# AsherBond/0-kno-vectorx

Hardware: AMD Instinct MI355X
Metric: header_range_256 proofs/sec (higher is better)
Workload: dtype u64 (Goldilocks) / u8 (hashes)

## Files before the change

### 0-kno-vectorx_amd/csrc/air.cuh

```cuda
#pragma once
#include <hip/hip_runtime.h>
#include <stdint.h>

#include <type_traits>
#include <vector>

#include "air_bus.cuh"
#include "gl.cuh"
#include "glh.h"

struct vx_ctx;
typedef int32_t (*gen_aux_fn)(vx_ctx*, const uint64_t* trace, int log_n, const uint64_t* chal, const uint64_t* pub, uint64_t* aux, uint64_t* aux_pub);

template <int R>
struct FpN {
    static constexpr int LANES = R;
    uint64_t v[R];
    __device__ __forceinline__ FpN operator+(const FpN& o) const {
        FpN r;
#pragma unroll
        for (int j = 0; j < R; ++j) r.v[j] = gl_add(v[j], o.v[j]);
        return r;
    }
    __device__ __forceinline__ FpN operator-(const FpN& o) const {
        FpN r;
#pragma unroll
        for (int j = 0; j < R; ++j) r.v[j] = gl_sub(v[j], o.v[j]);
        return r;
    }
    __device__ __forceinline__ FpN operator*(const FpN& o) const {
        FpN r;
#pragma unroll
        for (int j = 0; j < R; ++j) r.v[j] = gl_mul(v[j], o.v[j]);
        return r;
    }
// ... 47 lines not shown
        acc[0] = acc[0] * alpha[0] + c;
        acc[1] = acc[1] * alpha[1] + c;
    }
    VX_HD void transition(F c) { constraint(c * z_last); }
    VX_HD void first_row(F c) { constraint(c * l_first); }
    VX_HD void last_row(F c) { constraint(c * l_last); }
    VX_HD void constraint_x2(const X2<F>& e) {
        constraint(e.a);
        constraint(e.b);
    }
    VX_HD Gate open(F g) { return Gate{g}; }
    VX_HD void gated(Gate& G, F e) { constraint(G.g * e); }
    VX_HD void close(Gate&) {}
};

template <int R>
struct Consumer<FpN<R>> {
    using F = FpN<R>;
    struct Gate {
        gl_acc a0[R], a1[R];
        F g;
    };
    gl_acc acc0[R], acc1[R];
    const uint64_t* apow;
    int k;
    F z_last, l_first, l_last;
    __device__ __forceinline__ void init(const uint64_t* apow_) {
        apow = apow_, k = 0;
#pragma unroll
        for (int j = 0; j < R; ++j) gl_acc_zero(acc0[j]), gl_acc_zero(acc1[j]);
    }
    __device__ __forceinline__ void push(gl_acc* a0, gl_acc* a1, const F& c) {
        const int ku = __builtin_amdgcn_readfirstlane(k);
        const uint64_t p0 = apow[2 * ku], p1 = apow[2 * ku + 1];
#pragma unroll
        for (int j = 0; j < R; ++j) {
            gl_mac(a0[j], c.v[j], p0);
            gl_mac(a1[j], c.v[j], p1);
        }
        k = ku + 1;
    }
    __device__ __forceinline__ void constraint(const F& c) { push(acc0, acc1, c); }
    __device__ __forceinline__ void transition(const F& c) { constraint(c * z_last); }
    __device__ __forceinline__ void first_row(const F& c) { constraint(c * l_first); }
    __device__ __forceinline__ void last_row(const F& c) { constraint(c * l_last); }
    __device__ __forceinline__ void constraint_x2(const X2<F>& e) {
        constraint(e.a);
        constraint(e.b);
    }
    __device__ __forceinline__ Gate open(const F& g) {
        Gate G;
// ... 25 lines not shown
    int k = 0;
    void constraint(CountF) { ++k; }
    void transition(CountF) { ++k; }
    void first_row(CountF) { ++k; }
    void last_row(CountF) { ++k; }
    void constraint_x2(const X2<CountF>&) { k += 2; }
    Gate open(CountF) { return {}; }
    void gated(Gate&, CountF) { ++k; }
    void close(Gate&) {}
};
struct CountRow {
    CountF operator[](int) const { return {}; }
};

template <int R>
struct RowViewN {
    const uint64_t* base;
    size_t stride, i[R];
    __device__ __forceinline__ FpN<R> operator[](int col) const {
        const uint64_t* c = base + (size_t)col * stride;
        FpN<R> r;
#pragma unroll
        for (int j = 0; j < R; ++j) r.v[j] = c[i[j]];
        return r;
    }
};

template <class F, class Row, class Cn>
struct BusConstraints {
    static constexpr int UNROLL = 1;
    const Row& loc;
    Cn& c;
    int at;
    X2<F> hsum;
    VX_HD X2<F> helper() {
        const X2<F> h{loc[at], loc[at + 1]};
        at += 2, hsum = hsum + h;
        return h;
    }
    VX_HD void put(const F& ma, const X2<F>& da, const F& mb, const X2<F>& db) { c.constraint_x2(helper() * da * db - db * ma - da * mb); }
    VX_HD void pair(const F& m, const X2<F>& da, const X2<F>& db) { c.constraint_x2(helper() * da * db - (da + db) * m); }
    VX_HD void single(const F& m, const X2<F>& d) { c.constraint_x2(helper() * d - m); }
};
template <class Air, class F, class Row, class Cn>
VX_HD void bus_constraints(const Row& loc, const Row& nxt, const F* per, const F* pub, const F* chal, const F* apub, Cn& c) {
    static_assert(Air::AUX == 2 * Air::N_HELP + 2 && Air::AUXPUB == 1 && Air::CHAL == 4, "air.cuh: helpers, then one running sum");
// ... 62 lines not shown
```

### 0-kno-vectorx_amd/csrc/vx_core.hip

```cpp
#include <stdarg.h>
#include <stdlib.h>
#include <stdio.h>
#include <string.h>

#include "gl.cuh"
#include <dlfcn.h>

#include "vx_internal.h"

__attribute__((constructor)) static void vx_runtime_env() { setenv("GPU_MAX_HW_QUEUES", "16", 0); }

extern "C" int32_t vx_table_streams_mode(const char* table_streams, const char* hw_queues) {
    if (table_streams && strcmp(table_streams, "own") == 0) return VX_TABLE_STREAMS_OWN;
    if (table_streams && strcmp(table_streams, "shared") == 0) return VX_TABLE_STREAMS_SHARED;
    if (!hw_queues) return VX_TABLE_STREAMS_SHARED;
    char* end = nullptr;
    const long q = strtol(hw_queues, &end, 10);
    if (end == hw_queues || *end || q < 1) return VX_TABLE_STREAMS_OWN;
    return q <= 4 ? VX_TABLE_STREAMS_SHARED : VX_TABLE_STREAMS_OWN;
}

hipError_t vx_wait(vx_ctx* ctx) {
    if (ctx->table_streams != VX_TABLE_STREAMS_SHARED) return hipStreamSynchronize(ctx->stream);
    const hipError_t e = hipEventRecord(ctx->ev_wait, ctx->stream);
// ... 118 lines not shown
        ctx->scratch_n = n;
    }
    *out = ctx->scratch;
    return VX_OK;
}

extern "C" {

const char* vx_backend_name(void) { return "hip-gfx950"; }

static int32_t ctx_create(int device, vx_ctx* parent, vx_ctx** out) {
    if (!out) return VX_ERR_ARG;
    *out = nullptr;
    int n_dev = 0;
    if (hipGetDeviceCount(&n_dev) != hipSuccess || n_dev == 0 || device < 0 || device >= n_dev) return VX_ERR_DEVICE;
    vx_ctx* ctx = new vx_ctx();
    ctx->device = device;
    ctx->scratch = nullptr;
    ctx->scratch_n = 0;
    ctx->pinned = nullptr;
    ctx->pinned_n = 0;
    ctx->table_streams = parent ? parent->table_streams : vx_table_streams_mode(getenv("VX_TABLE_STREAMS"), getenv("GPU_MAX_HW_QUEUES"));
    ctx->stream_owned = !(parent && ctx->table_streams == VX_TABLE_STREAMS_SHARED);
    const char* sm = getenv("VX_SYNC_MODE");
    const char m = sm ? sm[0] : 'b';
    (void)hipSetDevice(device);
    (void)hipSetDeviceFlags(m == 's' ? hipDeviceScheduleSpin : m == 'y' ? hipDeviceScheduleYield : hipDeviceScheduleBlockingSync);
    (void)hipGetLastError();
    hipError_t se = hipSetDevice(device);
    if (se == hipSuccess && !ctx->stream_owned) ctx->stream = parent->stream;
    else if (se == hipSuccess) {
        const char* sp = getenv("VX_STREAM_PRIO");
        int least = 0, greatest = 0;
        if (sp && sp[0] == '1' && hipDeviceGetStreamPriorityRange(&least, &greatest) == hipSuccess && least != greatest)
            se = hipStreamCreateWithPriority(&ctx->stream, hipStreamDefault, parent ? least : greatest);
        else se = hipStreamCreate(&ctx->stream);
    }
    if (se != hipSuccess || hipEventCreate(&ctx->ev0) != hipSuccess || hipEventCreate(&ctx->ev1) != hipSuccess ||
        hipEventCreateWithFlags(&ctx->ev_wait, hipEventDisableTiming | (m == 's' || m == 'y' ? 0 : hipEventBlockingSync)) != hipSuccess) {
        delete ctx;
        return VX_ERR_DEVICE;
    }
    int32_t rc = make_powtab(ctx, glh::ROOT_2_32, &ctx->tw_fwd);
    if (rc == VX_OK) rc = make_powtab(ctx, glh::inv(glh::ROOT_2_32), &ctx->tw_inv);
    if (rc == VX_OK) {
        std::vector<uint64_t> f(2048), b(2048);
// ... 212 lines not shown
```

### 0-kno-vectorx_amd/csrc/vx_internal.h

```cpp
#pragma once
#include <hip/hip_runtime.h>
#include <stdint.h>
#include <map>
#include <string>
#include <vector>

#pragma GCC visibility push(default)
#include "../../include/vx.h"
#pragma GCC visibility pop
#include "glh.h"

#ifndef VX_TAIL_PRIO
#define VX_TAIL_PRIO 1
#endif
#if VX_TAIL_PRIO
#define VX_TAIL_KERNEL_ENTRY() __builtin_amdgcn_s_setprio(3)
#else
#define VX_TAIL_KERNEL_ENTRY() ((void)0)
#endif

struct vx_buf {
    uint64_t* d;
    size_t n;
};

struct PowTab {
    uint64_t* d;
};

enum { VX_TABLE_STREAMS_OWN = 0, VX_TABLE_STREAMS_SHARED = 1 };

struct vx_ctx {
    int device;
    hipStream_t stream;
    bool stream_owned;
    int table_streams;
    hipEvent_t ev0, ev1;
    hipEvent_t ev_wait;
    std::string err;
    PowTab tw_fwd, tw_inv;
    uint64_t *w12_fwd, *w12_inv;
    std::map<uint64_t, PowTab> shift_tabs;
    std::map<int, uint64_t*> tw2;
    uint64_t* scratch;
    size_t scratch_n;
    void* pinned;
    size_t pinned_n;
    std::map<size_t, std::vector<void*>> pool_free;
    std::map<void*, size_t> pool_live;
    vx_ctx* side = nullptr;
    std::map<uint64_t, uint64_t*> periodic_cache;
};
vx_ctx* vx_side_ctx(vx_ctx* ctx);
hipError_t vx_wait(vx_ctx* ctx);
void* vx_pool_alloc(vx_ctx* ctx, size_t bytes);
void vx_pool_free(vx_ctx* ctx, void* p);
void vx_pool_trim(vx_ctx* ctx);
int32_t vx_fail(vx_ctx* ctx, int32_t code, const char* fmt, ...);

// ... 118 lines not shown
```

### 0-kno-vectorx_amd/csrc/vx_stark.hip

```cpp
#include <string.h>

#include <map>
#include <mutex>

#include <array>

#include "air_list.h"
#include "air_program.h"
#include "bus_aux_prog.cuh"
#include "stark_proof.h"
#include "vx_internal.h"

namespace sp = stark_proof;

__device__ __forceinline__ uint64_t root_pow_f(const uint64_t* tw, uint64_t e, int log_s) {
    uint64_t E = (e << (32 - log_s)) & 0xFFFFFFFFULL;
    uint64_t r = tw[4096 + (E >> 22)];
    if (log_s > 10) r = gl_mul(r, tw[2048 + ((E >> 11) & 2047)]);
    if (log_s > 21) r = gl_mul(r, tw[E & 2047]);
    return r;
}

struct QuotArgs {
    const uint64_t* lde;
    uint64_t* q_out;
    int log_N, rate_bits;
    uint64_t shift, last, n_inv;
    uint64_t alpha[2];
    uint64_t zh_inv[8];
    uint64_t zh[8];
    const uint64_t* periodic;
    const uint64_t* pub;
    const uint64_t* tw;
    const uint64_t* apow;
    uint64_t chal[8];
    uint64_t apub[8];
};

#ifndef VX_Q_WAVES
#define VX_Q_WAVES 4
#endif
#ifndef VX_Q_WAVES_MAX
#define VX_Q_WAVES_MAX 8
#endif
#ifndef VX_Q_BLOCK
#define VX_Q_BLOCK 256
#endif
constexpr int QB = VX_Q_BLOCK;
template <class Air, int R>
__global__ __launch_bounds__(QB) __attribute__((amdgpu_waves_per_eu(VX_Q_WAVES, VX_Q_WAVES_MAX))) void k_quotient(QuotArgs a) {
    using F = FpN<R>;
    const size_t N = (size_t)1 << a.log_N;
    const size_t i0 = blockIdx.x * (size_t)(QB * R) + threadIdx.x;
    const size_t step = (size_t)1 << a.rate_bits;
    Consumer<F> c;
    c.init(a.apow);
    RowViewN<R> loc{a.lde, N, {}}, nxt{a.lde, N, {}};
    F per[Air::PERIODIC > 0 ? Air::PERIODIC : 1], pub[Air::PUB > 0 ? Air::PUB : 1];
    F chal[Air::CHAL > 0 ? Air::CHAL : 1], apub[Air::AUXPUB > 0 ? 2 * Air::AUXPUB : 1];
// ... 10 lines not shown
        zinv[j] = a.zh_inv[k];
        loc.i[j] = i;
        nxt.i[j] = (i + step) & (N - 1);
        size_t poff = 0;
#pragma unroll
        for (int q = 0; q < Air::PERIODIC; ++q) {
            const size_t plen = (size_t)1 << (Air::plog(q) + a.rate_bits);
            per[q].v[j] = a.periodic[poff + (i & (plen - 1))];
            poff += plen;
        }
    }
#pragma unroll
    for (int q = 0; q < Air::PUB; ++q) pub[q] = F::from(a.pub[q]);
#pragma unroll
    for (int q = 0; q < Air::CHAL; ++q) chal[q] = F::from(a.chal[q]);
#pragma unroll
    for (int q = 0; q < 2 * Air::AUXPUB; ++q) apub[q] = F::from(a.apub[q]);
    Air::template eval<F>(loc, nxt, per, pub, chal, apub, c);
#pragma unroll
    for (int j = 0; j < R; ++j) {
        a.q_out[loc.i[j]] = gl_mul(c.result(0, j), zinv[j]);
        a.q_out[N + loc.i[j]] = gl_mul(c.result(1, j), zinv[j]);
    }
}

struct ProgArgs {
    const uint64_t* code;
    const uint64_t* consts;
    const uint64_t* per_tab;
    int n_code;
};
__global__ __launch_bounds__(QB) void k_quotient_prog(QuotArgs a, ProgArgs p) {
    extern __shared__ uint64_t prog_regs[];
    using F = Fp;
    const size_t N = (size_t)1 << a.log_N;
    const size_t i = (blockIdx.x * (size_t)QB + threadIdx.x) & (N - 1);
    const size_t step = (size_t)1 << a.rate_bits, inext = (i + step) & (N - 1);
    Consumer<F> c;
    c.init(a.apow);
    const uint64_t x = gl_mul(a.shift, root_pow_f(a.tw, i, a.log_N));
    const int kz = (int)(i & (step - 1));
    c.z_last.v[0] = gl_sub(x, a.last);
    const uint64_t zh_n = gl_mul(a.zh[kz], a.n_inv);
    c.l_first.v[0] = gl_mul(zh_n, gl_inv(gl_sub(x, 1)));
    c.l_last.v[0] = gl_mul(gl_mul(zh_n, a.last), gl_inv(gl_sub(x, a.last)));
    uint64_t* R = prog_regs + threadIdx.x;
// ... 142 lines not shown
        const gl2 s1{gl_acc_reduce(sa[r]), gl_acc_reduce(sb[r])};
        gl2 s0 = s1;
        for (int j = 0; j < a.n_q; ++j) {
            const int k = a.n_cols + j;
            s0 = gl2_add(s0, gl2_scale({a.alpha_pow[2 * k], a.alpha_pow[2 * k + 1]}, a.quot_lde[(size_t)j * N + i]));
        }
        const uint64_t x = gl_mul(a.shift, root_pow_f(a.tw, i, a.log_N));
        gl2 t0 = gl2_mul(gl2_sub(s0, a.y0), gl2_inv({gl_sub(x, a.zeta.a), gl_neg(a.zeta.b)}));
        gl2 t1 = gl2_mul(gl2_sub(s1, a.y1), gl2_inv({gl_sub(x, a.zeta_next.a), gl_neg(a.zeta_next.b)}));
        gl2 f = gl2_add(gl2_mul(a.alpha_c, t0), t1);
        a.out[2 * i] = f.a;
        a.out[2 * i + 1] = f.b;
    }
}

struct AirDesc {
    int id, cols, pub, periodic, period_log, exact_log;
    void (*periodic_values)(std::vector<uint64_t>&);
    void (*launch)(QuotArgs&, hipStream_t);
    int (*count)();
    int aux, chal, auxpub;
    int (*plog)(int);
    gen_aux_fn gen_aux;
    const AirProgram* prog = nullptr;
};
template <class Air>
static int count_q() {
    static const int k = [] {
        Consumer<CountF> c;
        CountRow r;
        CountF per[Air::PERIODIC > 0 ? Air::PERIODIC : 1], pub[Air::PUB > 0 ? Air::PUB : 1], chal[Air::CHAL > 0 ? Air::CHAL : 1], apub[Air::AUXPUB > 0 ? 2 * Air::AUXPUB : 1];
        Air::template eval<CountF>(r, r, per, pub, chal, apub, c);
        return c.k;
    }();
    return k;
}
template <class Air>
static void launch_q(QuotArgs& a, hipStream_t s) {
    constexpr int R = Air::QUOT_ROWS_PER_LANE;
    const size_t N = (size_t)1 << a.log_N;
    if (R > 1 && N >= QB * (size_t)R) hipLaunchKernelGGL((k_quotient<Air, R>), dim3((unsigned)(N / (QB * R))), dim3(QB), 0, s, a);
    else hipLaunchKernelGGL((k_quotient<Air, 1>), dim3((unsigned)((N + QB - 1) / QB)), dim3(QB), 0, s, a);
}
template <class Air>
static AirDesc desc() {
    return {Air::ID, Air::COLS, Air::PUB, Air::PERIODIC, Air::PERIOD_LOG, Air::EXACT_LOG, Air::periodic_values, launch_q<Air>, count_q<Air>, Air::AUX, Air::CHAL, Air::AUXPUB, Air::plog, Air::gen_aux};
}
template <class... Airs>
static std::array<AirDesc, sizeof...(Airs)> descs(AirList<Airs...>) { return {{desc<Airs>()...}}; }
static const auto AIRS = descs(VxAirs{});
static std::mutex g_prog_desc_mu;
static std::map<int, AirDesc> g_prog_desc;
static const AirDesc* find_air(int id) {
    for (const AirDesc& d : AIRS)
        if (d.id == id) return &d;
    if (id >= VX_AIR_USER_BASE) {
        const AirProgram* pg = vx_air_program_find(id);
        if (!pg) return nullptr;
        std::lock_guard<std::mutex> lk(g_prog_desc_mu);
        auto it = g_prog_desc.find(id);
        if (it == g_prog_desc.end()) {
            AirDesc d{};
            d.id = id, d.cols = (int)pg->cols, d.pub = (int)pg->pub, d.periodic = (int)pg->plog.size(), d.period_log = pg->period_log, d.prog = pg;
            d.aux = (int)pg->aux, d.chal = (int)pg->chal, d.auxpub = (int)pg->auxpub;
            it = g_prog_desc.emplace(id, d).first;
        }
        return &it->second;
    }
    return nullptr;
// ... 56 lines not shown
}

struct DevMem;
static int32_t quotient_eval_dev(vx_ctx* ctx, const AirDesc* air, int L, int r, const uint64_t* trace_lde, const uint64_t alphas[2],
                                 const uint64_t* public_inputs, size_t n_public, const uint64_t* chal, const uint64_t* apub, uint64_t* qv, DevMem& mem);

extern "C" {

int32_t vx_stark_default_config(vx_stark_config* cfg) {
    if (!cfg) return VX_ERR_ARG;
    cfg->rate_bits = 1;
    cfg->cap_height = 4;
    cfg->num_queries = 84;
    cfg->pow_bits = 16;
    cfg->arity_bits = 4;
    cfg->final_poly_bits = 5;
    return VX_OK;
}

int32_t vx_stark_proof_bound(int air_id, const vx_stark_config* cfg, int log_n, size_t* n_words) {
    const AirDesc* air = find_air(air_id);
    if (!air || !cfg || !n_words || log_n < 2 || cfg->rate_bits < 1) return VX_ERR_ARG;
    *n_words = sp::Shape(air_id, air->cols, air->aux, air->pub, air->auxpub, log_n, *cfg).bound_words();
    return VX_OK;
}

int32_t vx_quotient_eval(vx_ctx* ctx, int air_id, int rate_bits, const vx_buf* trace_lde, int log_n, const uint64_t alphas[2],
                         const uint64_t* public_inputs, size_t n_public, vx_buf* out) {
    if (!ctx || !trace_lde || !alphas || !out) return VX_ERR_ARG;
    const AirDesc* air = find_air(air_id);
    VX_CHECK(air, "quotient eval: unknown AIR id %d", air_id);
    VX_CHECK(air->aux == 0, "quotient eval: AIR %d has an auxiliary round (its challenges are not part of this entry point)", air_id);
    VX_CHECK(rate_bits >= 1 && rate_bits <= 3 && log_n >= 2 && log_n >= air->period_log && log_n + rate_bits <= 27, "quotient eval: bad log_n %d / rate_bits %d", log_n, rate_bits);
    VX_CHECK((int)n_public == air->pub && (n_public == 0 || public_inputs), "quotient eval: AIR %d takes %d public inputs", air_id, air->pub);
    const size_t N = (size_t)1 << (log_n + rate_bits);
    VX_CHECK(trace_lde->n >= N * (size_t)air->cols && out->n >= 2 * N, "quotient eval: buffers too small");
    VX_CHECK(alphas[0] < glh::P && alphas[1] < glh::P, "quotient eval: non-canonical challenge");
    DevMem mem{ctx};
    return quotient_eval_dev(ctx, air, log_n, rate_bits, trace_lde->d, alphas, public_inputs, n_public, nullptr, nullptr, out->d, mem);
}

int32_t vx_quotient_eval_aux(vx_ctx* ctx, int air_id, int rate_bits, const vx_buf* trace_lde, int log_n, const uint64_t alphas[2],
                             const uint64_t* public_inputs, size_t n_public, const uint64_t* challenges, size_t n_challenges,
                             const uint64_t* aux_public, size_t n_aux_public, vx_buf* out) {
    if (!ctx || !trace_lde || !alphas || !out) return VX_ERR_ARG;
    const AirDesc* air = find_air(air_id);
// ... 65 lines not shown
        if (pl <= 6) {
            periodic_on_coset(pv.data() + in_off, pl, r, shift_pow, tab.data() + off);
            VX_HIP(hipMemcpyAsync(d + off, tab.data() + off, m * 8, hipMemcpyHostToDevice, ctx->stream));
        } else {
            uint64_t* tmp = (uint64_t*)vx_pool_alloc(ctx, p * 8);
            if (!tmp) {
                (void)hipFree(d);
                return vx_fail(ctx, VX_ERR_OOM, "stark prove: out of device memory (periodic table)");
            }
            VX_HIP(hipMemcpyAsync(tmp, pv.data() + in_off, p * 8, hipMemcpyHostToDevice, ctx->stream));
            int32_t rc = vx_lde_dev(ctx, tmp, pl, 1, r, shift_pow, VX_LDE_SRC_VALUES, d + off, nullptr);
            VX_HIP(vx_wait(ctx));
            vx_pool_free(ctx, tmp);
            if (rc != VX_OK) {
                (void)hipFree(d);
                return rc;
            }
        }
        off += m, in_off += p;
    }
    VX_HIP(vx_wait(ctx));
    ctx->periodic_cache[key] = d;
    *out = d;
    return VX_OK;
}

static int32_t quotient_eval_dev(vx_ctx* ctx, const AirDesc* air, int L, int r, const uint64_t* trace_lde, const uint64_t alphas[2],
                                 const uint64_t* public_inputs, size_t n_public, const uint64_t* chal, const uint64_t* apub, uint64_t* qv, DevMem& mem) {
    const int LN = L + r;
    const size_t n = (size_t)1 << L;
    const uint64_t g = 7;
    uint64_t* d_pub = mem.alloc(n_public ? n_public : 1);
    VX_CHECK(d_pub, "stark prove: out of device memory (quotient)");
    if (n_public) VX_HIP(hipMemcpyAsync(d_pub, public_inputs, n_public * 8, hipMemcpyHostToDevice, ctx->stream));
    const uint64_t* d_per = nullptr;
    if (air->periodic) VX_TRY(periodic_table_dev(ctx, air, L, r, &d_per));
    {
        QuotArgs qa{};
        qa.lde = trace_lde;
        qa.q_out = qv;
        qa.log_N = LN;
        qa.rate_bits = r;
        qa.shift = g;
        qa.last = glh::inv(glh::root(L));
        qa.n_inv = glh::inv(n % glh::P);
        qa.alpha[0] = alphas[0];
// ... 27 lines not shown
            uint64_t* d_code = nullptr;
            auto it = ctx->periodic_cache.find(key);
            if (it != ctx->periodic_cache.end()) d_code = it->second;
            else {
                std::vector<uint64_t> blob(pg.code);
                blob.insert(blob.end(), pg.consts.begin(), pg.consts.end());
                VX_HIP(hipMalloc((void**)&d_code, blob.size() * 8));
                VX_HIP(hipMemcpyAsync(d_code, blob.data(), blob.size() * 8, hipMemcpyHostToDevice, ctx->stream));
                VX_HIP(vx_wait(ctx));
                ctx->periodic_cache[key] = d_code;
            }
            size_t off = 0;
            for (size_t q = 0; q < pg.plog.size(); ++q) {
                const size_t plen = (size_t)1 << (pg.plog[q] + r);
                per_tab.push_back(off), per_tab.push_back(plen - 1);
                off += plen;
            }
            uint64_t* d_per_tab = mem.alloc(per_tab.size() ? per_tab.size() : 1);
            VX_CHECK(d_per_tab, "stark prove: out of device memory (program tables)");
            if (!per_tab.empty()) VX_HIP(hipMemcpyAsync(d_per_tab, per_tab.data(), per_tab.size() * 8, hipMemcpyHostToDevice, ctx->stream));
            ProgArgs pa{d_code, d_code + pg.code.size(), d_per_tab, (int)pg.code.size()};
            const size_t N = (size_t)1 << LN;
            hipLaunchKernelGGL(k_quotient_prog, dim3((unsigned)((N + QB - 1) / QB)), dim3(QB), pg.n_regs * QB * sizeof(uint64_t), ctx->stream, qa, pa);
        } else air->launch(qa, ctx->stream);
        VX_HIP(vx_wait(ctx));
        VX_HIP(hipGetLastError());
    }
    return VX_OK;
}

void vx_shared_challenges_n(const uint64_t* const* pubs, const size_t* n_pubs, const uint64_t* const* caps, size_t k, size_t cap_words, uint64_t* out, size_t n_out) {
    sp::shared_challenges_n(pubs, n_pubs, caps, k, cap_words, out, n_out);
}
void vx_shared_challenges(const uint64_t* pub_a, size_t n_a, const uint64_t* cap_a, const uint64_t* pub_b, size_t n_b, const uint64_t* cap_b,
                          size_t cap_words, uint64_t* out, size_t n_out) {
    const uint64_t *pubs[2] = {pub_a, pub_b}, *caps[2] = {cap_a, cap_b};
    const size_t ns[2] = {n_a, n_b};
    vx_shared_challenges_n(pubs, ns, caps, 2, cap_words, out, n_out);
}

int32_t vx_stark_prove_impl(vx_ctx* ctx, int air_id, const vx_stark_config* cfg_in, uint64_t* trace_d, size_t trace_len, int consume_trace,
                            int log_n, const uint64_t* public_inputs, size_t n_public, uint64_t* proof_out, size_t proof_cap,
                            size_t* proof_len, const vx_chal_hook* hook) {
    if (!ctx || !cfg_in || !trace_d || !proof_len) return VX_ERR_ARG;
    const AirDesc* air = find_air(air_id);
    VX_CHECK(air, "stark prove: unknown AIR id %d", air_id);
// ... 288 lines not shown
```

### 0-kno-vectorx_amd/lib.py

```python
import collections
import ctypes as C
import os
import subprocess

import numpy as np

_HERE = os.path.dirname(os.path.abspath(__file__))
LIB_PATH = os.environ.get("VX_LIB_PATH") or os.path.join(_HERE, "libvxprove.so")
P = 2**64 - 2**32 + 1

VX_ORDER_NATURAL, VX_ORDER_BITREV = 0, 1
VX_LDE_SRC_VALUES, VX_LDE_SRC_COEFFS = 0, 1
VX_LEAVES_ROW_MAJOR, VX_LEAVES_COLS_BITREV, VX_LEAVES_COLS = 0, 1, 2
ERR_NAMES = {-1: "VX_ERR_ARG", -2: "VX_ERR_DEVICE", -3: "VX_ERR_OOM", -4: "VX_ERR_BUFSZ", -5: "VX_ERR_STATEMENT", -6: "VX_ERR_POW"}

SYMBOLS = [
    "vx_ctx_create", "vx_ctx_destroy", "vx_sync", "vx_last_error", "vx_backend_name", "vx_timer_start", "vx_timer_stop", "vx_table_streams_mode",
    "vx_alloc", "vx_free", "vx_upload", "vx_download", "vx_copy", "vx_fill_random", "vx_buf_devptr", "vx_buf_len",
    "vx_field_batch_add", "vx_field_batch_sub", "vx_field_batch_mul", "vx_field_batch_inv", "vx_ext_batch_mul",
    "vx_ntt", "vx_lde", "vx_lde_rows",
    "vx_poseidon_permute_batch", "vx_merkle_build", "vx_merkle_free", "vx_merkle_cap", "vx_merkle_open", "vx_merkle_leaf_digests",
    "vx_fri_fold", "vx_fri_layer_tree", "vx_fri_leaves", "vx_fri_pow",
    "vx_stark_default_config", "vx_stark_proof_bound", "vx_stark_prove", "vx_stark_verify", "vx_header_range_proof_bound", "vx_header_range_prove", "vx_header_range_verify",
    "vx_header_range_proof_bound_ex", "vx_header_range_prove_ex", "vx_header_range_merge",
    "vx_blake2b_256_batch", "vx_sha256_pairs", "vx_verify_subchain", "vx_blake_chain_trace",
    "vx_ed25519_verify_batch", "vx_verify_simple_justification", "vx_sha_chain_trace",
    "vx_verify_epoch_end_header", "vx_rotate_proof_bound", "vx_rotate_prove", "vx_rotate_verify",
    "vx_gather_proofs", "vx_quotient_eval", "vx_quotient_eval_aux", "vx_decode_header_batch", "vx_decode_precommit_batch", "vx_stark_aux_trace",
    "vx_ed_trace", "vx_sha512_trace", "vx_epoch_end_trace", "vx_partial_products", "vx_air_register", "vx_air_register_bus", "vx_air_unregister", "vx_poseidon_air_trace",
    "vx_merkle_open_air_trace", "vx_merkle_openings_proof_bound", "vx_merkle_openings_prove", "vx_merkle_openings_verify",
    "vx_leaf_sponge_air_trace", "vx_merkle_rows_proof_bound", "vx_merkle_rows_prove", "vx_merkle_rows_verify",
    "vx_fri_fold_air_trace", "vx_fri_fold_proof_bound", "vx_fri_fold_prove", "vx_fri_fold_verify", "vx_stark_fri_claims",
    "vx_merkle_open_set_air_trace", "vx_leaf_sponge_set_air_trace", "vx_fri_queries_proof_bound", "vx_fri_queries_prove", "vx_fri_queries_verify",
    "vx_fri_combine_air_trace", "vx_fri_combine_proof_bound", "vx_fri_combine_prove", "vx_fri_combine_verify", "vx_stark_combine_claims",
    "vx_fri_combine_fold_proof_bound", "vx_fri_combine_fold_prove", "vx_fri_combine_fold_verify",
    "vx_stark_merkle_claims", "vx_merkle_paths_air_trace", "vx_leaf_sponge_rows_air_trace", "vx_stark_openings_proof_bound", "vx_stark_openings_prove", "vx_stark_openings_verify",
    "vx_leaf_noop_air_trace", "vx_stark_queries_proof_bound", "vx_stark_queries_prove", "vx_stark_queries_verify", "vx_stark_proof_head_words",
    "vx_transcript_air_trace", "vx_stark_transcript_claims", "vx_stark_transcripts_proof_bound", "vx_stark_transcripts_prove", "vx_stark_transcripts_verify",
    "vx_stark_inner_proof_bound", "vx_stark_inner_prove", "vx_stark_inner_verify",
    "vx_bus_group_proof_bound", "vx_bus_group_prove", "vx_bus_group_verify", "vx_bus_group_check",
]

VX_AIR_FIBONACCI, VX_AIR_MIX, VX_AIR_BLAKE_CHAIN, VX_AIR_LOOKUP = 1, 2, 6, 5
VX_BLAKE_AIR_COLS, VX_BLAKE_AIR_AUX_COLS = 745, 276
VX_AIR_SHA_TREE = {256: 7, 512: 8, 16: 9}
VX_AIR_SHA_CHAIN, VX_SHA_AIR_COLS, VX_SHA_AIR_AUX_COLS, VX_SHA_TREE_AIR_COLS = 4, 414, 4, 412
VX_AIR_ED25519 = {17: 10, 16: 12}
VX_ED_AIR_COLS, VX_ED_AIR_AUX_COLS = 839, 688
VX_AIR_SHA512 = {16: 11, 15: 14, 10: 13}
VX_SHA512_AIR_COLS, VX_SHA512_AIR_AUX_COLS = 801, 4
VX_AIR_EPOCH_END, VX_EPOCH_END_AIR_COLS, VX_EPOCH_END_AIR_AUX_COLS = 15, 52, 46
# ... 726 lines not shown
        idx = np.ascontiguousarray(idx, dtype=np.uint64)
        out = np.empty((idx.size, self.depth, 4), dtype=np.uint64)
        self.ctx._ck(self.ctx.L.vx_merkle_open(self.ctx.h, self.h, _ptr(idx), idx.size, _ptr(out)))
        return out

    def leaf_digests(self):
        out = np.empty((self.n_leaves, 4), dtype=np.uint64)
        self.ctx._ck(self.ctx.L.vx_merkle_leaf_digests(self.ctx.h, self.h, _ptr(out)))
        return out

    def free(self):
        if self.h:
            self.ctx.L.vx_merkle_free(self.ctx.h, self.h)
            self.h = None


def table_streams_mode(table_streams, hw_queues):
    f = load_library().vx_table_streams_mode
    f.argtypes, f.restype = [C.c_char_p, C.c_char_p], C.c_int32
    a, b = (None if v is None else str(v).encode() for v in (table_streams, hw_queues))
    return ("own", "shared")[f(a, b)]


class Context:

    def __init__(self, device=0):
        self.L = load_library()
        h = C.c_void_p()
        rc = self.L.vx_ctx_create(device, C.byref(h))
        if rc != 0:
            raise VxError(rc, f"vx_ctx_create(device={device}) failed: no usable gfx950 device (no CPU fallback exists)")
        self.h = h

    def _ck(self, rc):
        if rc != 0:
            raise VxError(rc, self.L.vx_last_error(self.h).decode())

    @classmethod
    def adopt(cls, handle):
        c = cls.__new__(cls)
        c.L, c.h, c.borrowed = load_library(), C.c_void_p(handle), True
        return c

    def close(self):
        if self.h and not getattr(self, "borrowed", False):
            self.L.vx_ctx_destroy(self.h)
# ... 517 lines not shown
```

### include/vx.h

```cpp
#ifndef VX_H
#define VX_H
#include <stddef.h>
#include <stdint.h>
#ifdef __cplusplus
extern "C" {
#endif

typedef struct vx_ctx vx_ctx;
typedef struct vx_buf vx_buf;
typedef struct vx_tree vx_tree;

enum {
    VX_OK = 0,
    VX_ERR_ARG = -1,
    VX_ERR_DEVICE = -2,
    VX_ERR_OOM = -3,
    VX_ERR_BUFSZ = -4,
    VX_ERR_STATEMENT = -5,
    VX_ERR_POW = -6
};

int32_t vx_ctx_create(int device, vx_ctx** out);
int32_t vx_ctx_destroy(vx_ctx* ctx);
int32_t vx_sync(vx_ctx* ctx);
// ... 196 lines not shown
typedef struct vx_bus_expect {
    int32_t air_id;
    const uint64_t* public_inputs;
    size_t n_public;
} vx_bus_expect;
typedef struct vx_bus_unmatched {
    uint64_t n_unmatched;
    int32_t table;
    uint32_t message;
    uint64_t row;
    uint64_t net;
} vx_bus_unmatched;
int32_t vx_bus_group_proof_bound(const vx_stark_config* cfg, const vx_bus_table* tables, size_t n, size_t* n_words);
int32_t vx_bus_group_prove(vx_ctx* ctx, const vx_stark_config* cfg, const vx_bus_table* tables, size_t n, const uint64_t* outside, size_t n_outside, uint64_t* blob_out,
                           size_t blob_cap, size_t* blob_len);
int32_t vx_bus_group_verify(const vx_stark_config* cfg, const uint64_t* blob, size_t blob_len, const vx_bus_expect* expect, size_t n, const uint64_t* outside, size_t n_outside,
                            char* err, size_t errlen);
int32_t vx_bus_group_check(vx_ctx* ctx, const vx_bus_table* tables, size_t n, const uint64_t* outside, size_t n_outside, vx_bus_unmatched* out);
int32_t vx_quotient_eval(vx_ctx* ctx, int air_id, int rate_bits, const vx_buf* trace_lde, int log_n, const uint64_t alphas[2],
                         const uint64_t* public_inputs, size_t n_public, vx_buf* out);
int32_t vx_quotient_eval_aux(vx_ctx* ctx, int air_id, int rate_bits, const vx_buf* trace_lde, int log_n, const uint64_t alphas[2],
                             const uint64_t* public_inputs, size_t n_public, const uint64_t* challenges, size_t n_challenges,
                             const uint64_t* aux_public, size_t n_aux_public, vx_buf* out);
int32_t vx_partial_products(vx_ctx* ctx, const vx_buf* wires, const vx_buf* sigmas, int log_n, size_t n_routed, const uint64_t* k_is,
                            uint64_t beta, uint64_t gamma, size_t chunk, vx_buf* out);
int32_t vx_stark_aux_trace(vx_ctx* ctx, int air_id, const vx_buf* trace, int log_n, const uint64_t* public_inputs, size_t n_public,
                           const uint64_t* challenges, size_t n_challenges, vx_buf* aux_out, uint64_t* aux_public_out);
int32_t vx_stark_proof_bound(int air_id, const vx_stark_config* cfg, int log_n, size_t* n_words);
int32_t vx_stark_prove(vx_ctx* ctx, int air_id, const vx_stark_config* cfg, const vx_buf* trace, int log_n,
                       const uint64_t* public_inputs, size_t n_public, uint64_t* proof_out, size_t proof_cap,
                       size_t* proof_len);
int32_t vx_stark_verify(const vx_stark_config* cfg, const uint64_t* proof, size_t proof_len, int expect_air,
                        const uint64_t* expect_public, size_t n_expect_public, char* err, size_t errlen);

int32_t vx_blake2b_256_batch(vx_ctx* ctx, const vx_buf* msgs, size_t stride, const uint32_t* sizes, size_t n,
                             uint8_t* digests_out);
int32_t vx_sha256_pairs(vx_ctx* ctx, const uint8_t* pairs64, size_t n, uint8_t* out32);

enum { VX_AIR_BLAKE_CHAIN = 6, VX_BLAKE_AIR_COLS = 745, VX_BLAKE_AIR_AUX_COLS = 276 };
int32_t vx_blake_chain_trace(vx_ctx* ctx, const vx_buf* headers, size_t stride, const uint32_t* sizes, size_t n_headers,
                             const uint8_t trusted_hash[32], uint32_t first_block_number, uint32_t tree_size, uint32_t window_offset, uint32_t window_length,
                             int log_n, vx_buf* trace_out, uint64_t public_inputs_out[20], uint8_t* digests_out);

enum { VX_AIR_SHA_CHAIN = 4, VX_SHA_AIR_COLS = 414, VX_SHA_AIR_AUX_COLS = 4, VX_SHA_TREE_AIR_COLS = 412  };
int32_t vx_sha_chain_trace(vx_ctx* ctx, const uint8_t* pubkeys, size_t n_keys, const uint8_t* signed_flags, uint32_t bus_on, int log_n, vx_buf* trace_out,
                           uint64_t public_inputs_out[10], uint8_t commitment_out[32]);
// ... 80 lines not shown
```

Before: 9.028.

## Stage quotient trace reads through an LDS ring driven by a precomputed access schedule

Adds a staged quotient kernel. On the host, the AIR constraint evaluation is recorded once to get the exact order of column reads. On the device, those reads are prefetched with global_load_lds into a 16-slot per-wave LDS ring, using explicit vmcnt waits, so many trace loads are in flight ahead of the constraint arithmetic. The kernel is enabled by default for the Blake, SHA, Ed25519 and related AIRs. The alpha-power pointer is also moved to the constant address space so it can be loaded with scalar loads. The risks are LDS use that may lower occupancy, hand-written waitcnt ordering, and extra schedule memory.

```diff
diff --git a/0-kno-vectorx_amd/csrc/air.cuh b/0-kno-vectorx_amd/csrc/air.cuh
--- a/0-kno-vectorx_amd/csrc/air.cuh
+++ b/0-kno-vectorx_amd/csrc/air.cuh
@@ -11,6 +11,8 @@
 
 struct vx_ctx;
 typedef int32_t (*gen_aux_fn)(vx_ctx*, const uint64_t* trace, int log_n, const uint64_t* chal, const uint64_t* pub, uint64_t* aux, uint64_t* aux_pub);
+
+#define VX_AS(n) __attribute__((address_space(n)))
 
 template <int R>
 struct FpN {
@@ -104,11 +106,11 @@
         F g;
     };
     gl_acc acc0[R], acc1[R];
-    const uint64_t* apow;
+    const VX_AS(4) uint64_t* apow;
     int k;
     F z_last, l_first, l_last;
     __device__ __forceinline__ void init(const uint64_t* apow_) {
-        apow = apow_, k = 0;
+        apow = (const VX_AS(4) uint64_t*)apow_, k = 0;
 #pragma unroll
         for (int j = 0; j < R; ++j) gl_acc_zero(acc0[j]), gl_acc_zero(acc1[j]);
     }
@@ -180,6 +182,64 @@
         FpN<R> r;
 #pragma unroll
         for (int j = 0; j < R; ++j) r.v[j] = c[i[j]];
+        return r;
+    }
+};
+
+struct SchedRow {
+    std::vector<uint32_t>* rec;
+    uint32_t next;
+    CountF operator[](int col) const {
+        rec->push_back((uint32_t)col << 1 | next);
+        return {};
+    }
+};
+
+#ifndef VX_Q_RING
+#define VX_Q_RING 16
+#endif
+constexpr int Q_RING = VX_Q_RING;
+static_assert(Q_RING >= 2 && Q_RING <= 64 && (Q_RING & (Q_RING - 1)) == 0, "air.cuh: the ring is a power of two of slots, and vmcnt counts to 63");
+struct StagedRing {
+    const VX_AS(4) uint32_t* sched;
+    int k;
+    uint32_t e_next;
+    const char* lde;
+    int log_N;
+    uint32_t off[2];
+    bool lo;
+    VX_AS(3) char* ring;
+    uint32_t lane8;
+#ifdef VX_Q_CHECK_ORDER
+    uint32_t* err;
+#endif
+    __device__ __forceinline__ void fetch(uint32_t e, int slot) const {
+        const char* src = lde + ((size_t)(e >> 1) << (log_N + 3)) + ((e & 1) ? off[1] : off[0]);
+        if (lo) __builtin_amdgcn_global_load_lds((const VX_AS(1) void*)src, (VX_AS(3) void*)(ring + slot * 512), 16, 0, 0);
+    }
+    __device__ __forceinline__ void start() {
+#pragma unroll
+        for (int j = 0; j < Q_RING - 1; ++j) fetch(sched[j], j);
+        e_next = sched[Q_RING - 1], k = 0;
+    }
+};
+struct StagedRow {
+    StagedRing* st;
+    uint32_t next;
+    __device__ __forceinline__ FpN<1> operator[](int col) const {
+        StagedRing& s = *st;
+        const int k = __builtin_amdgcn_readfirstlane(s.k);
+        const uint32_t e = __builtin_amdgcn_readfirstlane(s.e_next);
+        asm volatile("s_waitcnt lgkmcnt(0)" ::: "memory");
+        s.fetch(e, (k - 1) & (Q_RING - 1));
+        s.e_next = s.sched[k + Q_RING];
+#ifdef VX_Q_CHECK_ORDER
+        if (s.sched[k] != ((uint32_t)col << 1 | next)) atomicMin(s.err, (uint32_t)k);
+#endif
+        asm volatile("s_waitcnt vmcnt(%0)" ::"n"(Q_RING - 1) : "memory");
+        FpN<1> r;
+        r.v[0] = *(const VX_AS(3) uint64_t*)(s.ring + (k & (Q_RING - 1)) * 512 + s.lane8);
+        s.k = k + 1;
         return r;
     }
 };
diff --git a/0-kno-vectorx_amd/csrc/vx_core.hip b/0-kno-vectorx_amd/csrc/vx_core.hip
--- a/0-kno-vectorx_amd/csrc/vx_core.hip
+++ b/0-kno-vectorx_amd/csrc/vx_core.hip
@@ -164,6 +164,8 @@
     ctx->pinned_n = 0;
     ctx->table_streams = parent ? parent->table_streams : vx_table_streams_mode(getenv("VX_TABLE_STREAMS"), getenv("GPU_MAX_HW_QUEUES"));
     ctx->stream_owned = !(parent && ctx->table_streams == VX_TABLE_STREAMS_SHARED);
+    const char* qs = parent ? nullptr : getenv("VX_Q_STAGED");
+    ctx->q_staged = parent ? parent->q_staged : qs && strcmp(qs, "0") == 0 ? VX_Q_STAGED_OFF : qs && strcmp(qs, "1") == 0 ? VX_Q_STAGED_ON : VX_Q_STAGED_AUTO;
     const char* sm = getenv("VX_SYNC_MODE");
     const char m = sm ? sm[0] : 'b';
     (void)hipSetDevice(device);
diff --git a/0-kno-vectorx_amd/csrc/vx_internal.h b/0-kno-vectorx_amd/csrc/vx_internal.h
--- a/0-kno-vectorx_amd/csrc/vx_internal.h
+++ b/0-kno-vectorx_amd/csrc/vx_internal.h
@@ -29,12 +29,14 @@
 };
 
 enum { VX_TABLE_STREAMS_OWN = 0, VX_TABLE_STREAMS_SHARED = 1 };
+enum { VX_Q_STAGED_OFF = 0, VX_Q_STAGED_ON = 1, VX_Q_STAGED_AUTO = 2 };
 
 struct vx_ctx {
     int device;
     hipStream_t stream;
     bool stream_owned;
     int table_streams;
+    int q_staged;
     hipEvent_t ev0, ev1;
     hipEvent_t ev_wait;
     std::string err;
diff --git a/0-kno-vectorx_amd/csrc/vx_stark.hip b/0-kno-vectorx_amd/csrc/vx_stark.hip
--- a/0-kno-vectorx_amd/csrc/vx_stark.hip
+++ b/0-kno-vectorx_amd/csrc/vx_stark.hip
@@ -35,6 +35,8 @@
     const uint64_t* apow;
     uint64_t chal[8];
     uint64_t apub[8];
+    const uint32_t* sched;
+    uint32_t* sched_err;
 };
 
 #ifndef VX_Q_WAVES
@@ -91,6 +93,54 @@
         a.q_out[loc.i[j]] = gl_mul(c.result(0, j), zinv[j]);
         a.q_out[N + loc.i[j]] = gl_mul(c.result(1, j), zinv[j]);
     }
+}
+
+template <class Air>
+__global__ __launch_bounds__(QB) __attribute__((amdgpu_waves_per_eu(VX_Q_WAVES, VX_Q_WAVES_MAX))) void k_quotient_staged(QuotArgs a) {
+    __shared__ uint64_t ring[QB / 64][Q_RING * 64];
+    using F = Fp;
+    const size_t N = (size_t)1 << a.log_N;
+    const size_t step = (size_t)1 << a.rate_bits;
+    const uint32_t lane = threadIdx.x & 63, wave = __builtin_amdgcn_readfirstlane(threadIdx.x >> 6);
+    const size_t i = (blockIdx.x * (size_t)QB + threadIdx.x) & (N - 1);
+    StagedRing st;
+    st.sched = (const VX_AS(4) uint32_t*)a.sched, st.lde = (const char*)a.lde, st.log_N = a.log_N;
+    const size_t at = ((blockIdx.x * (size_t)QB + wave * 64) & (N - 1)) + 2 * (lane & 31);
+    st.off[0] = (uint32_t)(at * 8), st.off[1] = (uint32_t)(((at + step) & (N - 1)) * 8);
+    st.lo = lane < 32, st.ring = (VX_AS(3) char*)&ring[wave][0], st.lane8 = lane * 8;
+#ifdef VX_Q_CHECK_ORDER
+    st.err = a.sched_err;
+#endif
+    st.start();
+    Consumer<F> c;
+    c.init(a.apow);
+    F per[Air::PERIODIC > 0 ? Air::PERIODIC : 1], pub[Air::PUB > 0 ? Air::PUB : 1];
+    F chal[Air::CHAL > 0 ? Air::CHAL : 1], apub[Air::AUXPUB > 0 ? 2 * Air::AUXPUB : 1];
+    const uint64_t x = gl_mul(a.shift, root_pow_f(a.tw, i, a.log_N));
+    const int kz = (int)(i & (step - 1));
+    c.z_last.v[0] = gl_sub(x, a.last);
+    const uint64_t zh_n = gl_mul(a.zh[kz], a.n_inv);
+    c.l_first.v[0] = gl_mul(zh_n, gl_inv(gl_sub(x, 1)));
+    c.l_last.v[0] = gl_mul(gl_mul(zh_n, a.last), gl_inv(gl_sub(x, a.last)));
+    const uint64_t zinv = a.zh_inv[kz];
+    size_t poff = 0;
+#pragma unroll
+    for (int q = 0; q < Air::PERIODIC; ++q) {
+        const size_t plen = (size_t)1 << (Air::plog(q) + a.rate_bits);
+        per[q].v[0] = a.periodic[poff + (i & (plen - 1))];
+        poff += plen;
+    }
+#pragma unroll
+    for (int q = 0; q < Air::PUB; ++q) pub[q] = F::from(a.pub[q]);
+#pragma unroll
+    for (int q = 0; q < Air::CHAL; ++q) chal[q] = F::from(a.chal[q]);
+#pragma unroll
+    for (int q = 0; q < 2 * Air::AUXPUB; ++q) apub[q] = F::from(a.apub[q]);
+    const StagedRow loc{&st, 0}, nxt{&st, 1};
+    [[clang::always_inline]] Air::template eval<F>(loc, nxt, per, pub, chal, apub, c);
+    a.q_out[i] = gl_mul(c.result(0, 0), zinv);
+    a.q_out[N + i] = gl_mul(c.result(1, 0), zinv);
+    asm volatile("s_waitcnt vmcnt(0)" ::: "memory");
 }
 
 struct ProgArgs {
@@ -279,6 +329,9 @@
     int aux, chal, auxpub;
     int (*plog)(int);
     gen_aux_fn gen_aux;
+    const std::vector<uint32_t>& (*sched)() = nullptr;
+    void (*launch_staged)(QuotArgs&, hipStream_t) = nullptr;
+    bool staged_auto = false;
     const AirProgram* prog = nullptr;
 };
 template <class Air>
@@ -293,6 +346,35 @@
     return k;
 }
 template <class Air>
+static const std::vector<uint32_t>& sched_q() {
+    static const std::vector<uint32_t> v = [] {
+        std::vector<uint32_t> rec;
+        Consumer<CountF> c;
+        const SchedRow loc{&rec, 0}, nxt{&rec, 1};
+        CountF per[Air::PERIODIC > 0 ? Air::PERIODIC : 1], pub[Air::PUB > 0 ? Air::PUB : 1], chal[Air::CHAL > 0 ? Air::CHAL : 1], apub[Air::AUXPUB > 0 ? 2 * Air::AUXPUB : 1];
+        Air::template eval<CountF>(loc, nxt, per, pub, chal, apub, c);
+        return rec;
+    }();
+    return v;
+}
+template <class Air>
+struct QuotStagedAuto : std::false_type {};
+template <>
+struct QuotStagedAuto<BlakeAir> : std::true_type {};
+template <>
+struct QuotStagedAuto<ShaAir> : std::true_type {};
+template <int LOGN, int ID_>
+struct QuotStagedAuto<EdAirT<LOGN, ID_>> : std::true_type {};
+template <int LOGN, int ID_>
+struct QuotStagedAuto<Sha512AirT<LOGN, ID_>> : std::true_type {};
+template <int LOGN, int ID_>
+struct QuotStagedAuto<ShaTreeAirT<LOGN, ID_>> : std::true_type {};
+template <class Air>
+static void launch_q_staged(QuotArgs& a, hipStream_t s) {
+    const size_t N = (size_t)1 << a.log_N;
+    hipLaunchKernelGGL((k_quotient_staged<Air>), dim3((unsigned)((N + QB - 1) / QB)), dim3(QB), 0, s, a);
+}
+template <class Air>
 static void launch_q(QuotArgs& a, hipStream_t s) {
     constexpr int R = Air::QUOT_ROWS_PER_LANE;
     const size_t N = (size_t)1 << a.log_N;
@@ -301,7 +383,8 @@
 }
 template <class Air>
 static AirDesc desc() {
-    return {Air::ID, Air::COLS, Air::PUB, Air::PERIODIC, Air::PERIOD_LOG, Air::EXACT_LOG, Air::periodic_values, launch_q<Air>, count_q<Air>, Air::AUX, Air::CHAL, Air::AUXPUB, Air::plog, Air::gen_aux};
+    return {Air::ID, Air::COLS, Air::PUB, Air::PERIODIC, Air::PERIOD_LOG, Air::EXACT_LOG, Air::periodic_values, launch_q<Air>, count_q<Air>, Air::AUX, Air::CHAL, Air::AUXPUB, Air::plog, Air::gen_aux,
+            sched_q<Air>, Air::QUOT_ROWS_PER_LANE == 1 ? launch_q_staged<Air> : nullptr, QuotStagedAuto<Air>::value};
 }
 template <class... Airs>
 static std::array<AirDesc, sizeof...(Airs)> descs(AirList<Airs...>) { return {{desc<Airs>()...}}; }
@@ -404,6 +487,15 @@
     const AirDesc* air = find_air(air_id);
     if (!air || !cfg || !n_words || log_n < 2 || cfg->rate_bits < 1) return VX_ERR_ARG;
     *n_words = sp::Shape(air_id, air->cols, air->aux, air->pub, air->auxpub, log_n, *cfg).bound_words();
+    return VX_OK;
+}
+
+int32_t vx_air_access_schedule(int air_id, uint32_t* out, size_t cap, size_t* len) {
+    const AirDesc* air = find_air(air_id);
+    if (!air || !air->sched || !len || (cap && !out)) return VX_ERR_ARG;
+    const std::vector<uint32_t>& sc = air->sched();
+    *len = sc.size();
+    for (size_t k = 0; k < sc.size() && k < cap; ++k) out[k] = sc[k];
     return VX_OK;
 }
 
@@ -515,6 +607,29 @@
     VX_HIP(vx_wait(ctx));
     ctx->periodic_cache[key] = d;
     *out = d;
+    return VX_OK;
+}
+
+static bool staged_wanted(const vx_ctx* ctx, const AirDesc* air, int LN, const uint64_t* lde) {
+    if (air->prog || !air->launch_staged || !air->sched) return false;
+    if (!(ctx->q_staged == VX_Q_STAGED_ON || (ctx->q_staged == VX_Q_STAGED_AUTO && air->staged_auto))) return false;
+    return LN >= 6 && !air->sched().empty() && ((uintptr_t)lde & 15) == 0;
+}
+static int32_t schedule_dev(vx_ctx* ctx, const AirDesc* air, const uint32_t** out) {
+    const uint64_t key = ((uint64_t)air->id << 16) | 0xFFFEULL;
+    auto it = ctx->periodic_cache.find(key);
+    if (it != ctx->periodic_cache.end()) {
+        *out = (const uint32_t*)it->second;
+        return VX_OK;
+    }
+    std::vector<uint32_t> padded(air->sched());
+    padded.resize(padded.size() + Q_RING, 0);
+    uint64_t* d = nullptr;
+    VX_HIP(hipMalloc((void**)&d, padded.size() * 4));
+    VX_HIP(hipMemcpyAsync(d, padded.data(), padded.size() * 4, hipMemcpyHostToDevice, ctx->stream));
+    VX_HIP(vx_wait(ctx));
+    ctx->periodic_cache[key] = d;
+    *out = (const uint32_t*)d;
     return VX_OK;
 }
 
@@ -588,6 +703,20 @@
             ProgArgs pa{d_code, d_code + pg.code.size(), d_per_tab, (int)pg.code.size()};
             const size_t N = (size_t)1 << LN;
             hipLaunchKernelGGL(k_quotient_prog, dim3((unsigned)((N + QB - 1) / QB)), dim3(QB), pg.n_regs * QB * sizeof(uint64_t), ctx->stream, qa, pa);
+        } else if (staged_wanted(ctx, air, LN, trace_lde)) {
+            VX_TRY(schedule_dev(ctx, air, &qa.sched));
+#ifdef VX_Q_CHECK_ORDER
+            qa.sched_err = (uint32_t*)mem.alloc(1);
+            VX_CHECK(qa.sched_err, "stark prove: out of device memory (schedule check)");
+            VX_HIP(hipMemsetAsync(qa.sched_err, 0xFF, 8, ctx->stream));
+#endif
+            air->launch_staged(qa, ctx->stream);
+#ifdef VX_Q_CHECK_ORDER
+            uint32_t first = 0;
+            VX_HIP(hipMemcpyAsync(&first, qa.sched_err, 4, hipMemcpyDeviceToHost, ctx->stream));
+            VX_HIP(vx_wait(ctx));
+            VX_CHECK(first == 0xFFFFFFFFu, "quotient of AIR %d: access %u reads another column than the schedule names", air->id, first);
+#endif
         } else air->launch(qa, ctx->stream);
         VX_HIP(vx_wait(ctx));
         VX_HIP(hipGetLastError());
diff --git a/0-kno-vectorx_amd/lib.py b/0-kno-vectorx_amd/lib.py
--- a/0-kno-vectorx_amd/lib.py
+++ b/0-kno-vectorx_amd/lib.py
@@ -26,7 +26,7 @@
     "vx_blake2b_256_batch", "vx_sha256_pairs", "vx_verify_subchain", "vx_blake_chain_trace",
     "vx_ed25519_verify_batch", "vx_verify_simple_justification", "vx_sha_chain_trace",
     "vx_verify_epoch_end_header", "vx_rotate_proof_bound", "vx_rotate_prove", "vx_rotate_verify",
-    "vx_gather_proofs", "vx_quotient_eval", "vx_quotient_eval_aux", "vx_decode_header_batch", "vx_decode_precommit_batch", "vx_stark_aux_trace",
+    "vx_gather_proofs", "vx_quotient_eval", "vx_quotient_eval_aux", "vx_air_access_schedule", "vx_decode_header_batch", "vx_decode_precommit_batch", "vx_stark_aux_trace",
     "vx_ed_trace", "vx_sha512_trace", "vx_epoch_end_trace", "vx_partial_products", "vx_air_register", "vx_air_register_bus", "vx_air_unregister", "vx_poseidon_air_trace",
     "vx_merkle_open_air_trace", "vx_merkle_openings_proof_bound", "vx_merkle_openings_prove", "vx_merkle_openings_verify",
     "vx_leaf_sponge_air_trace", "vx_merkle_rows_proof_bound", "vx_merkle_rows_prove", "vx_merkle_rows_verify",
@@ -799,6 +799,20 @@
     return ("own", "shared")[f(a, b)]
 
 
+def air_access_schedule(air_id):
+    f = load_library().vx_air_access_schedule
+    f.argtypes, f.restype = [C.c_int, C.c_void_p, C.c_size_t, C.c_void_p], C.c_int32
+    n = C.c_size_t(0)
+    rc = f(air_id, None, 0, C.byref(n))
+    if rc != 0:
+        raise VxError(rc, "vx_air_access_schedule: AIR %d has no compiled constraints" % air_id)
+    out = np.zeros(max(n.value, 1), dtype=np.uint32)
+    rc = f(air_id, out.ctypes.data_as(C.c_void_p), n.value, C.byref(n))
+    if rc != 0:
+        raise VxError(rc, "vx_air_access_schedule failed")
+    return [(int(e) >> 1, int(e) & 1) for e in out[:n.value]]
+
+
 class Context:
 
     def __init__(self, device=0):
diff --git a/include/vx.h b/include/vx.h
--- a/include/vx.h
+++ b/include/vx.h
@@ -242,6 +242,7 @@
 int32_t vx_quotient_eval_aux(vx_ctx* ctx, int air_id, int rate_bits, const vx_buf* trace_lde, int log_n, const uint64_t alphas[2],
                              const uint64_t* public_inputs, size_t n_public, const uint64_t* challenges, size_t n_challenges,
                              const uint64_t* aux_public, size_t n_aux_public, vx_buf* out);
+int32_t vx_air_access_schedule(int air_id, uint32_t* out, size_t cap, size_t* len);
 int32_t vx_partial_products(vx_ctx* ctx, const vx_buf* wires, const vx_buf* sigmas, int log_n, size_t n_routed, const uint64_t* k_is,
                             uint64_t beta, uint64_t gamma, size_t chunk, vx_buf* out);
 int32_t vx_stark_aux_trace(vx_ctx* ctx, int air_id, const vx_buf* trace, int log_n, const uint64_t* public_inputs, size_t n_public,
```

New measurement: 9.066 (median of 6 runs). Within noise of the previous version (+0.4%).
